# damians13/big-linear-algebra

Hardware: AMD Instinct MI355X
Metric: fp32 GFLOP/s matrix_mul 4096^3 (higher is better)
Workload: dtype f32; 1 GPU; square fp32 matrix_multiply N=4096 (BASELINE configs[1]), operands resident in HBM; kernel=gemm_f32_glds256x256x16_nn_dma_splitk1, parallelism=replicas x1

## Files before the change

big-linear-algebra_amd/csrc/bla_gemm.hip:

```cpp

#include "bla_gemm_kernel.h"

namespace bla {

enum { LOAD_FULL = 0, LOAD_VEC = 1, LOAD_SCALAR = 2 };

template <int ROWS, int COLS, int NT>
struct TileRegs {
	static constexpr int CPR = COLS / 4;
	static constexpr int N = ROWS * COLS / 4 / NT;
	static_assert(ROWS * COLS / 4 % NT == 0, "tile must divide over the workgroup");
	float4 v[N];

	template <int MODE>
	__device__ __forceinline__ void load(const float* __restrict__ g, int ld, int row0, int col0, int row_end, int col_end, int tid) {
#pragma unroll
		for (int i = 0; i < N; i++) {
			int f = tid + i * NT;
			int gr = row0 + f / CPR, gc = col0 + (f % CPR) * 4;
			if (MODE == LOAD_FULL) {
				v[i] = *reinterpret_cast<const float4*>(g + (size_t)gr * ld + gc);
			} else if (MODE == LOAD_VEC) {
				bool ok = gr < row_end && gc < col_end;
				const float* q = g + (size_t)min(gr, row_end - 1) * ld + min(gc, col_end - 4);
// ... 683 lines not shown
			void* ws;
			st = ensure_workspace((size_t)wtiles * ksplit * 1024 * sizeof(float), &ws);
			if (st) return st;
			a.slab = (float*)ws;
		}
		dim3 grid((unsigned)wtiles, (unsigned)ksplit);
		if (plan && ksplit == 1 && avec && bvec) { plan->a = a; plan->akc = akc; plan->bkc = bkc; plan->valid = true; return BLA_OK; }
		hipError_t e = launch_wsk(a, akc, bkc, avec, bvec, grid, s);
		if (e != hipSuccess) return hip_fail(e, "gemm_f32_wsk_kernel launch");
		snprintf(g_last_kernel, sizeof(g_last_kernel), "gemm_f32_wsk%dx%d_%c%c_%s%s_ksplit%d", tile, tile, transa ? 't' : 'n', transb ? 't' : 'n',
		         avec ? "v" : "s", bvec ? "v" : "s", ksplit);
		return BLA_OK;
	}
	BLA_REQUIRE(!a.softmax_grad || cfg == 6, BLA_ERR_INVALID, "fused softmax is only available on the wave-split-K config (6)");
	float* deferred_row_sum = nullptr;
	BLA_REQUIRE(cfg == 6 || !a.row_sum_a || (a.rs_alpha == 1.f && a.rs_beta == 0.f), BLA_ERR_INVALID, "a scaled / accumulated row sum is only available on the wave-split-K config (6)");
	if (cfg != 6 && a.row_sum_a) { deferred_row_sum = a.row_sum_a; a.row_sum_a = nullptr; }
	if (kConfigs[cfg].glds && !(vec_ok && k > 0 && k % kConfigs[cfg].bk == 0)) {
		set_error("gemm config %d (%s) needs 16-byte aligned operands, contiguous extents %% 4 == 0 and k %% %d == 0", cfg,
		          kConfigs[cfg].name, kConfigs[cfg].bk);
		return BLA_ERR_INVALID;
	}
	const Config& c = kConfigs[cfg];
	a.tiles_m = (m + c.bm - 1) / c.bm;
	a.tiles_n = (n + c.bn - 1) / c.bn;
	long tiles = (long)a.tiles_m * a.tiles_n;
	int splits = g_force_split;
	if (splits <= 0) {
		splits = 1;
		if (tiles < cus && k >= 256) {
			long want = (2L * cus + tiles - 1) / tiles;
			long maxs = k / 128;
			splits = (int)(want < maxs ? want : maxs);
			if (splits < 1) splits = 1;
			if (splits > 32) splits = 32;
		}
	}
	if ((cfg >= 11 && cfg <= 15) || cfg == kCfgHs192) {
		BLA_REQUIRE(m % c.bm == 0 && n % c.bn == 0 && k >= 2 * c.bk && ldc % 4 == 0 && (uintptr_t)C % 16 == 0, BLA_ERR_INVALID,
		            "gemm config %d (%s) needs m, n multiples of the tile, k >= %d and a 16-byte aligned C", cfg, c.name, 2 * c.bk);
		a.rc_global = 0;
		BLA_REQUIRE(!a.bias_row && !a.bias_col && !a.pre_act && a.act == BLA_ACT_NONE && !a.relu_mask && a.beta == 0.f && !deferred_row_sum, BLA_ERR_INVALID,
		            "gemm config %d (%s) takes a plain epilogue (alpha only)", cfg, c.name);
		splits = 1;
	}
	if (cfg == 10) {
		BLA_REQUIRE(k % (2 * c.bk) == 0, BLA_ERR_INVALID, "gemm config 10 (%s) needs k %% %d == 0", c.name, 2 * c.bk);
		splits = 1;
	}
	int kps = (k + splits - 1) / splits;
	kps = (kps + c.bk - 1) / c.bk * c.bk;
	if (kps == 0) kps = c.bk;
	splits = k > 0 ? (k + kps - 1) / kps : 1;
	a.k_per_split = kps;
	a.splits = splits;
	a.slab = nullptr;
	if (splits > 1) {
		void* ws;
		st = ensure_workspace((size_t)splits * m * n * sizeof(float), &ws);
		if (st) return st;
		a.slab = (float*)ws;
	}
	int mode = LOAD_SCALAR;
	if (vec_ok) {
		mode = LOAD_VEC;
		if (m % c.bm == 0 && n % c.bn == 0 && k % c.bk == 0) mode = LOAD_FULL;
	}
	dim3 grid((unsigned)tiles, 1, (unsigned)splits);
	hipError_t e;
	switch (cfg) {
		case 0: e = launch_variant<128, 128, 16, 2, 2>(a, akc, bkc, mode, grid, s); break;
		case 1: e = launch_variant<64, 64, 16, 2, 2>(a, akc, bkc, mode, grid, s); break;
		case 2: e = launch_variant<128, 128, 32, 2, 2>(a, akc, bkc, mode, grid, s); break;
		case 3: e = launch_glds<128, 128, 16, 2, 2>(a, akc, bkc, grid, s); break;
		case 4: e = launch_glds<64, 64, 16, 2, 2>(a, akc, bkc, grid, s); break;
		case 5: e = launch_glds<128, 128, 32, 2, 2>(a, akc, bkc, grid, s); break;
		case 7: e = launch_glds<128, 64, 16, 2, 2>(a, akc, bkc, grid, s); break;
		case 8: e = launch_glds<128, 256, 16, 2, 2, 2, 3>(a, akc, bkc, grid, s); break;
		case 9: e = launch_glds<256, 128, 16, 2, 2, 2, 3>(a, akc, bkc, grid, s); break;
		case 10: {
			unsigned tiles = grid.x, cap = 2u * (unsigned)cus;
			e = launch_glds<128, 128, 16, 2, 2, 1, 2, true>(a, akc, bkc, dim3(tiles < cap ? tiles : cap, 1, 1), s);
		} break;
		case 11: e = launch_glds<256, 256, 16, 2, 2>(a, akc, bkc, grid, s); break;
		case 12: e = launch_glds<256, 256, 32, 2, 2>(a, akc, bkc, grid, s); break;
		case 13: e = launch_glds<128, 512, 16, 1, 4>(a, akc, bkc, grid, s); break;
		case 14: e = launch_glds<128, 128, 16, 2, 2, 1, 2, false, true>(a, akc, bkc, grid, s); break;
		case 15: e = launch_glds<128, 256, 16, 2, 2, 1, 2, false, true>(a, akc, bkc, grid, s); break;
		case 18: e = launch_glds<64, 64, 32, 2, 2, 1, 2, false, false, 2>(a, akc, bkc, grid, s); break;
		default: e = launch_glds<192, 192, 16, 2, 2, 1, 2, false, true>(a, akc, bkc, grid, s); break;
	}
	if (e != hipSuccess) return hip_fail(e, "gemm_f32_kernel launch");
	static const char* kModeName[] = {"full", "vec", "scalar"};
	snprintf(g_last_kernel, sizeof(g_last_kernel), "gemm_f32_%s_%c%c_%s_splitk%d", c.name, transa ? 't' : 'n', transb ? 't' : 'n',
	         c.glds ? "dma" : kModeName[mode], splits);
	if (splits > 1) {
		e = launch_splitk_reduce(a, s);
		if (e != hipSuccess) return hip_fail(e, "gemm_splitk_reduce_kernel launch");
	}
	if (deferred_row_sum) return window_sum(stream, A, m, k, lda, deferred_row_sum);
	return BLA_OK;
}

extern "C" {

bla_status bla_gemm_f32(void* stream, int transa, int transb, int m, int n, int k,
                        const float* A, int lda, const float* B, int ldb, float* C, int ldc,
                        const bla_gemm_epilogue* ep) {
	return gemm_impl(stream, transa, transb, m, n, k, A, lda, B, ldb, C, ldc, ep, nullptr);
}

bla_status bla_gemm_pair_f32(void* stream, const bla_gemm_desc* p, const bla_gemm_desc* q) { return gemm_pair_with_hook(stream, p, q, nullptr, nullptr); }

}

bla_status bla::gemm_pair_with_hook(void* stream, const bla_gemm_desc* p, const bla_gemm_desc* q, const DoneHook* d_hook, bool* posted) {
	if (posted) *posted = false;
	BLA_REQUIRE(p && q, BLA_ERR_INVALID, "null descriptor");
	WskPlan pp = {}, pq = {};
	const bool try_pair = g_force_config < 0 && g_force_split <= 0;
	bla_status st = gemm_impl(stream, p->transa, p->transb, p->m, p->n, p->k, p->A, p->lda, p->B, p->ldb, p->C, p->ldc, p->ep, try_pair ? &pp : nullptr);
	if (st) return st;
	st = gemm_impl(stream, q->transa, q->transb, q->m, q->n, q->k, q->A, q->lda, q->B, q->ldb, q->C, q->ldc, q->ep, pp.valid ? &pq : nullptr);
	if (st) return st;
	hipStream_t s = pick_stream(stream);
	const int tp = pp.valid ? pp.a.tiles_m * pp.a.tiles_n : 0, tq = pq.valid ? pq.a.tiles_m * pq.a.tiles_n : 0;
	hipError_t e = hipSuccess;
	if (pp.valid && pq.valid && !pp.a.softmax_grad && !pq.a.softmax_grad) {
		const dim3 grid((unsigned)(tp + tq));
		const int combo = (pp.akc ? 8 : 0) | (pp.bkc ? 4 : 0) | (pq.akc ? 2 : 0) | (pq.bkc ? 1 : 0);
#define BLA_PAIR_CASE(I) case I: hipLaunchKernelGGL((gemm_f32_wsk_pair_kernel<((I) & 8) != 0, ((I) & 4) != 0, ((I) & 2) != 0, ((I) & 1) != 0>), grid, dim3(256), 0, s, pp.a, pq.a, tp, d_hook); break
		switch (combo) {
			BLA_PAIR_CASE(0); BLA_PAIR_CASE(1); BLA_PAIR_CASE(2); BLA_PAIR_CASE(3); BLA_PAIR_CASE(4); BLA_PAIR_CASE(5); BLA_PAIR_CASE(6); BLA_PAIR_CASE(7);
			BLA_PAIR_CASE(8); BLA_PAIR_CASE(9); BLA_PAIR_CASE(10); BLA_PAIR_CASE(11); BLA_PAIR_CASE(12); BLA_PAIR_CASE(13); BLA_PAIR_CASE(14); BLA_PAIR_CASE(15);
		}
#undef BLA_PAIR_CASE
		e = hipGetLastError();
		if (posted && e == hipSuccess) *posted = d_hook != nullptr;
		snprintf(g_last_kernel, sizeof(g_last_kernel), "gemm_f32_wsk_pair_%c%c+%c%c_%dx%d+%dx%d", pp.akc ? 'n' : 't', pp.bkc ? 't' : 'n', pq.akc ? 'n' : 't',
		         pq.bkc ? 't' : 'n', tp, pp.a.wsk_tile, tq, pq.a.wsk_tile);
	} else {
		if (pp.valid) e = launch_wsk(pp.a, pp.akc, pp.bkc, true, true, dim3((unsigned)tp, 1), s);
		if (e == hipSuccess && pq.valid) e = launch_wsk(pq.a, pq.akc, pq.bkc, true, true, dim3((unsigned)tq, 1), s);
	}
	if (e != hipSuccess) return hip_fail(e, "gemm_f32_wsk pair launch");
	return BLA_OK;
}

extern "C" {

bla_status bla_gemm_batched_f32(void* stream, int transa, int transb, int m, int n, int k, const float* A, int lda, long stride_a, const float* B, int ldb,
                                long stride_b, float* C, int ldc, long stride_c, int batch, const bla_gemm_epilogue* ep, long stride_pre) {
	BLA_REQUIRE(batch >= 1, BLA_ERR_INVALID, "batch %d", batch);
	BLA_REQUIRE(!ep || (!ep->relu_mask && !ep->row_sum_a && !ep->softmax_grad), BLA_ERR_INVALID, "batched products take alpha / beta, the biases, act and pre_act only");
	if (batch == 1) return gemm_impl(stream, transa, transb, m, n, k, A, lda, B, ldb, C, ldc, ep, nullptr);
	if (g_force_config < 0 && g_force_split <= 0 && gemm_thin_applies(m, n, k, batch) && (!ep || (!ep->bias_col && ep->act == BLA_ACT_NONE))) {
		BLA_REQUIRE(A && B && C, BLA_ERR_INVALID, "null operand");
		const ThinPart part = {A, B, stride_a, stride_b, lda, ldb};
		bla_status st = gemm_thin_parts(stream, transa, transb, m, n, k, &part, 1, C, ldc, stride_c, batch, ep ? ep->alpha : 1.f, ep ? ep->beta : 0.f,
		                                ep ? ep->bias_row : nullptr, ep ? ep->pre_act : nullptr, ep ? ep->ld_pre : 0, stride_pre);
		if (st == BLA_OK) snprintf(g_last_kernel, sizeof(g_last_kernel), "gemm_f32_thin_%c%c_x%d", transa ? 't' : 'n', transb ? 't' : 'n', batch);
		return st;
	}
	WskPlan pl = {};
	const bool aligned = stride_a % 4 == 0 && stride_b % 4 == 0 && stride_c % 4 == 0 && stride_pre % 4 == 0;
	t_plan_batch = batch;
	bla_status st = gemm_impl(stream, transa, transb, m, n, k, A, lda, B, ldb, C, ldc, ep, g_force_config < 0 && g_force_split <= 0 && aligned ? &pl : nullptr);
// ... 58 lines not shown
```

big-linear-algebra_amd/csrc/bla_gemm_kernel.h:

```cpp
#pragma once
#include "bla_internal.h"
#include <cstdlib>

namespace bla {

typedef float f32x16 __attribute__((ext_vector_type(16)));

struct GemmArgs {
	const float* A; const float* B; float* C;
	int M, N, K, lda, ldb, ldc;
	int tiles_m, tiles_n, k_per_split, splits;
	float* slab;
	float alpha, beta;
	const float* bias_row; const float* bias_col;
	float* pre_act; int ld_pre; int act;
	const float* relu_mask; int ld_mask;
#ifdef BLA_WSK_DIAG
	unsigned long long* stamps;
#endif
	unsigned* counters;
	float* row_sum_a;
	float rs_alpha, rs_beta;
	const float* softmax_y; float softmax_scale; float* softmax_grad;
	double* sm_loss; unsigned* sm_correct;
// ... 264 lines not shown
		if (GATHER == 3) {
#pragma unroll
			for (int i = 0; i < B_NI; i++) {
				const int idx = wave * B_NI + i, kr = idx * 2 + (lane >> 5);
				const float* src = p.g_img + (g3_base + p.g_ktab[g_k + kr].x);
				__builtin_amdgcn_global_load_lds((gbl_ptr_t)src, (lds_ptr_t)(base + A_SZ + idx * 256), 16, 0, 0);
			}
			g_k += BK;
		} else if (GATHER) {
			const int simg = GATHER == 2 ? g_img * p.g_img_stride : 0;
#pragma unroll
			for (int i = 0; i < B_NI; i++) {
				const int idx = wave * B_NI + i, krow = idx >> 1, hf = idx & 1;
				const int2 ts = p.g_ktab[GATHER == 1 ? g_k + krow : g_r + krow];
				const int yy = (short)(g_lyx[hf] & 0xffff) + (short)(ts.y & 0xffff), xx = (g_lyx[hf] >> 16) + (ts.y >> 16);
				const bool ok = g_lval[hf] && (unsigned)yy < (unsigned)p.g_H && (unsigned)xx < (unsigned)p.g_W;
				const float* src = ok ? p.g_img + (g_loff[hf] + ts.x + simg) : p.g_zero;
				__builtin_amdgcn_global_load_lds((gbl_ptr_t)src, (lds_ptr_t)(base + A_SZ + krow * BN + hf * 64), 4, 0, 0);
			}
			g_k += BK;
			if (GATHER == 2) {
				g_r += BK;
				if (g_r >= p.g_HWo) {
					g_r = 0; g_img++;
#pragma unroll
					for (int i = 0; i < A_NI; i++) ga[i] += (size_t)(p.M - 1) * p.g_HWo;
				}
			}
		} else {
#pragma unroll
			for (int i = 0; i < B_NI; i++) {
				__builtin_amdgcn_global_load_lds((gbl_ptr_t)gb[i], (lds_ptr_t)(base + A_SZ + (wave * B_NI + i) * 256), 16, 0, 0);
				gb[i] += b_step;
			}
		}
	};

	f32x16 acc[TM][TN];
#pragma unroll
	for (int i = 0; i < TM; i++)
#pragma unroll
		for (int j = 0; j < TN; j++)
#pragma unroll
			for (int r = 0; r < 16; r++) acc[i][j][r] = 0.f;

	auto frags = [&](const float* As, const float* Bs, int kk, float (&a)[TM][4], float (&b)[TN][4]) {
#pragma unroll
		for (int i = 0; i < TM; i++) {
			if (AKC) {
				float4 x = *reinterpret_cast<const float4*>(As + AI::off(wm0 + i * 32 + l31, kk * 2 + h));
				a[i][0] = x.x; a[i][1] = x.y; a[i][2] = x.z; a[i][3] = x.w;
			} else {
#pragma unroll
				for (int j = 0; j < 4; j++) a[i][j] = As[(kk * 8 + 4 * h + j) * BM + wm0 + i * 32 + l31];
			}
		}
#pragma unroll
		for (int i = 0; i < TN; i++) {
			if (BKC) {
				float4 x = *reinterpret_cast<const float4*>(Bs + BI::off(wn0 + i * 32 + l31, kk * 2 + h));
				b[i][0] = x.x; b[i][1] = x.y; b[i][2] = x.z; b[i][3] = x.w;
			} else {
#pragma unroll
				for (int j = 0; j < 4; j++) b[i][j] = Bs[(kk * 8 + 4 * h + j) * BN + wn0 + i * 32 + l31];
			}
		}
	};

	auto mfma_group = [&](float (&a)[KKW][TM][4], float (&b)[KKW][TN][4], int kk, int j) {
#pragma unroll
		for (int im = 0; im < TM; im++)
#pragma unroll
			for (int in = 0; in < TN; in++)
				acc[im][in] = __builtin_amdgcn_mfma_f32_32x32x2f32(a[kk][im][j], b[kk][in][j], acc[im][in], 0, 0, 0);
	};
	auto rest = [&](float (&pa)[KKW][TM][4], float (&pb)[KKW][TN][4]) {
#pragma unroll
		for (int kk = 0; kk < KKW; kk++)
#pragma unroll
			for (int j = 0; j < 4; j++)
				if (kk != 0 || j != 0) mfma_group(pa, pb, kk, j);
	};
	constexpr bool HALFSLAB = ((TM == 4 && TN == 4) || (HS && TM >= 2 && TM <= 4 && TN >= 2 && TN <= 4)) && (KK == 2 || KK == 4) &&
	                          (GATHER == 0 || ((GATHER == 3 || GATHER == 4 || G7) && HS)) && !PERSIST && NBUF == 2;
	constexpr int NDMA = G7 ? A_NI + 1 : A_NI + B_NI;
	size_t g_adv_a = 0, g_adv_b = 0;
	int w7_tap = 0, w7_g = 0;
	const int w7_groups = G7 ? (p.g_img_stride / p.g_HWo) / 16 : 0, w7_gstep = 16 * p.g_HWo;
	const float* const w7_img = p.g_img;
	const float* const w7_zero = p.g_zero;
#if defined(__HIP_DEVICE_COMPILE__)
	int hs_tap[B_NI][2];
	auto hs_prefetch = [&]() {
		if (GATHER == 3) {
#pragma unroll
			for (int i = 0; i < B_NI; i++) {
				const int row = __builtin_amdgcn_readfirstlane(g_k + (wave * B_NI + i) * G3_RPI);
				hs_tap[i][0] = p.g_ktab[row].x; hs_tap[i][1] = G3_RPI == 2 ? p.g_ktab[row + 1].x : 0;
			}
		}
	};
	if (HALFSLAB && GATHER == 3) hs_prefetch();

	auto dma_one = [&](int buf, int d) {
		float* base = lds + buf * (A_SZ + B_SZ);
		if (d < A_NI) {
			const int i = d;
			if (GATHER == 4) {
				__builtin_amdgcn_raw_ptr_buffer_load_lds(rsrc_img, (lds_ptr_t)(base + (wave * A_NI + i) * 256), 16, g4_voff[i], g4_soff, 0, 0);
			} else if (A_BUF) __builtin_amdgcn_raw_ptr_buffer_load_lds(rsrc_a, (lds_ptr_t)(base + (wave * A_NI + i) * 256), 16, voff_a[i], soff_a, 0, 0);
			else __builtin_amdgcn_global_load_lds((gbl_ptr_t)(ga[i] + g_adv_a), (lds_ptr_t)(base + (wave * A_NI + i) * 256), 16, 0, 0);
		} else if (G7) {
			if (w7_tap < W7_PW && wave + 4 * w7_tap < W7_NI && w7_g + 1 < w7_groups) {
				const int i = w7_tap;
				const int off = window_chunk_offset<W7_PL, GWS>((wave + 4 * i) * 64 + lane, w7_i0, p.g_H, p.g_HWo, w7_base);
				const float* src = off >= 0 ? w7_img + (off + (w7_g + 1) * w7_gstep) : w7_zero;
				float* dst = lds + 2 * A_SZ + 4 + ((w7_g + 1) & 1) * W7_GRP + (wave + 4 * i) * 256;
				__builtin_amdgcn_global_load_lds((gbl_ptr_t)src, (lds_ptr_t)dst, 16, 0, 0);
			}
		} else {
			const int i = d - A_NI;
			if (GATHER == 3) {
				const int idx = wave * B_NI + i;
				const float* src = p.g_img + (g3_base + ((G3_RPI == 2 && (lane >> 5)) ? hs_tap[i][1] : hs_tap[i][0]));
				__builtin_amdgcn_global_load_lds((gbl_ptr_t)src, (lds_ptr_t)(base + A_SZ + idx * 256), 16, 0, 0);
			} else if (B_BUF) __builtin_amdgcn_raw_ptr_buffer_load_lds(rsrc_b, (lds_ptr_t)(base + A_SZ + (wave * B_NI + i) * 256), 16, voff_b[i], soff_b, 0, 0);
			else __builtin_amdgcn_global_load_lds((gbl_ptr_t)(gb[i] + g_adv_b), (lds_ptr_t)(base + A_SZ + (wave * B_NI + i) * 256), 16, 0, 0);
		}
	};
	auto dma_advance = [&](bool really) {
		const int sa = really ? (int)(a_step * 4) : 0, sb = really ? (int)(b_step * 4) : 0;
		if (GATHER == 3) { soff_a += sa; g_k += really ? BK : 0; hs_prefetch(); return; }
		if (G7) { soff_a += sa; return; }
		if (GATHER == 4) {
			const int r1 = g_r + (really ? BK : 0);
			const bool wrap = r1 >= p.g_HWo;
			soff_b += (really ? BK * 4 : 0) + (wrap ? (p.N - 1) * p.g_HWo * 4 : 0);
			g_r = wrap ? 0 : r1; g_img += wrap ? 1 : 0;
			const int c1 = g4_col + 16;
			const bool row_end = c1 >= p.g_wo;
			g4_pix0 = wrap ? 0 : g4_pix0 + (really ? (row_end ? g4_step_end : g4_step) : 0);
			g4_col = (wrap || row_end) ? 0 : (really ? c1 : g4_col);
			g4_soff = __builtin_amdgcn_readfirstlane((g_img * p.g_img_stride + g4_pix0) * 4);
			return;
		}
		if (A_BUF) soff_a += sa; else g_adv_a += really ? a_step : 0;
		if (B_BUF) soff_b += sb; else g_adv_b += really ? b_step : 0;
	};
#else
	auto dma_one = [&](int, int) {};
	auto dma_advance = [&](bool) {};
#endif
	auto step = [&](int kt, bool do_dma, float (&pa)[KKW][TM][4], float (&pb)[KKW][TN][4], float (&qa)[KKW][TM][4], float (&qb)[KKW][TN][4]) {
		mfma_group(pa, pb, 0, 0);
		__builtin_amdgcn_sched_barrier(0);
		asm volatile("s_waitcnt vmcnt(0)" ::: "memory");
		__builtin_amdgcn_s_barrier();
		const float* As = lds + ((kt + 1) & 1) * (A_SZ + B_SZ);
#pragma unroll
		for (int kk = 0; kk < KKW; kk++) frags(As, As + A_SZ, wk * KKW + kk, qa[kk], qb[kk]);
		if (do_dma) dma(kt & 1);
		__builtin_amdgcn_sched_barrier(0);
		rest(pa, pb);
		__builtin_amdgcn_sched_barrier(0);
	};

	auto store_tile = [&]() {
		if (GATHER == 4) {
			float* dst = p.splits > 1 ? p.slab + (size_t)zsplit * p.M * p.N : p.C;
			const int ld = p.splits > 1 ? p.M : p.ldc;
#pragma unroll
			for (int in = 0; in < TN; in++) {
				int col = n0 + wn0 + in * 32 + l31;
				if (col >= p.N) continue;
#pragma unroll
				for (int im = 0; im < TM; im++)
#pragma unroll
					for (int qq = 0; qq < 4; qq++) {
						int row = m0 + wm0 + im * 32 + 8 * qq + 4 * h;
						if (row + 3 < p.M)
							*reinterpret_cast<float4*>(dst + (size_t)col * ld + row) =
								make_float4(acc[im][in][4 * qq], acc[im][in][4 * qq + 1], acc[im][in][4 * qq + 2], acc[im][in][4 * qq + 3]);
					}
			}
			return;
		}
		if constexpr (G7) {
			const int b = n0 / p.g_HWo;
			const size_t img_off = (size_t)b * p.M * p.g_HWo + (n0 - b * p.g_HWo) + wn0 + l31;
			const float* bias = p.g_bias ? p.g_bias + (size_t)b * p.g_bias_stride : nullptr;
#pragma unroll
			for (int im = 0; im < TM; im++)
#pragma unroll
				for (int r = 0; r < 16; r++) {
					const int row = m0 + wm0 + im * 32 + (r & 3) + 8 * (r >> 2) + 4 * h;
					const size_t o = img_off + (size_t)row * p.g_HWo;
					const float bv = bias ? bias[row] : 0.f;
#pragma unroll
					for (int in = 0; in < TN; in++) {
						const float v = acc[im][in][r] + bv;
						p.C[o + in * 32] = v;
						if (p.g_out2) p.g_out2[o + in * 32] = v + p.g_add[o + in * 32];
					}
				}
			return;
		}
		if constexpr (GATHER == 3 && HALFSLAB) {
			const int col = n0 + wn0 + TN * l31;
			const int b = col / p.g_HWo, rr = col - b * p.g_HWo;
			const size_t img_off = (size_t)b * p.M * p.g_HWo + rr;
			float* cbase = (p.splits > 1 ? p.slab + (size_t)zsplit * p.M * p.N : p.C) + img_off;
			const float* bias = p.g_bias ? p.g_bias + (size_t)b * p.g_bias_stride : nullptr;
#pragma unroll
			for (int im = 0; im < TM; im++)
#pragma unroll
				for (int r = 0; r < 16; r++) {
					const int row = m0 + wm0 + im * 32 + (r & 3) + 8 * (r >> 2) + 4 * h;
					const size_t o = (size_t)row * p.g_HWo;
					const float bv = bias ? bias[row] : 0.f;
					if (TN == 4) {
						const float4 v = make_float4(acc[im][0][r] + bv, acc[im][1][r] + bv, acc[im][TN > 2 ? 2 : 0][r] + bv, acc[im][TN > 3 ? 3 : 0][r] + bv);
						*reinterpret_cast<float4*>(cbase + o) = v;
						if (p.g_out2) {
							const float4 a4 = *reinterpret_cast<const float4*>(p.g_add + img_off + o);
							*reinterpret_cast<float4*>(p.g_out2 + img_off + o) = make_float4(v.x + a4.x, v.y + a4.y, v.z + a4.z, v.w + a4.w);
						}
					} else {
						const float2 v = make_float2(acc[im][0][r] + bv, acc[im][1][r] + bv);
						*reinterpret_cast<float2*>(cbase + o) = v;
						if (p.g_out2) {
							const float2 a2 = *reinterpret_cast<const float2*>(p.g_add + img_off + o);
							*reinterpret_cast<float2*>(p.g_out2 + img_off + o) = make_float2(v.x + a2.x, v.y + a2.y);
						}
					}
				}
			return;
		}
		if (GATHER == 1 || GATHER == 3) {
#pragma unroll
			for (int in = 0; in < TN; in++) {
				int col = n0 + wn0 + in * 32 + l31;
				if (col >= p.N) continue;
				int b = col / p.g_HWo, r = col - b * p.g_HWo;
				float* cbase = p.C + (size_t)b * p.M * p.g_HWo + r;
#pragma unroll
				for (int im = 0; im < TM; im++)
#pragma unroll
					for (int q = 0; q < 16; q++) {
						int row = m0 + wm0 + im * 32 + (q & 3) + 8 * (q >> 2) + 4 * h;
// ... 162 lines not shown
					__builtin_amdgcn_sched_barrier(0);
#pragma unroll
					for (int m = FRONT ? u : u * NM / NU; m < (FRONT ? (u + 1 < NU ? u + 1 : NM) : (u + 1) * NM / NU); m++) mf1(use, m);
					__builtin_amdgcn_sched_barrier(0);
				}
			}
			land(Q);
			asm volatile("s_waitcnt vmcnt(0)" ::: "memory");
			__builtin_amdgcn_s_barrier();
#if defined(__HIP_DEVICE_COMPILE__)
			if constexpr (GATHER == 3) {
#pragma unroll
				for (int i = 0; i < B_NI; i++) { asm volatile("" : "+v"(hs_tap[i][0])); if (G3_RPI == 2) asm volatile("" : "+v"(hs_tap[i][1])); }
			}
#endif
			constexpr int PER = 2 * (NU + NDMA) <= NM ? 2 : 1;
			static_assert(PER * (NU + NDMA) <= NM, "too many memory instructions for the MFMAs of one k-part");
#pragma unroll
			for (int u = 0; u < NU; u++) {
				read_unit(nxt, 0, u, P);
				__builtin_amdgcn_sched_barrier(0);
#pragma unroll
				for (int m = 0; m < PER; m++) mf1(Q, PER * u + m);
				__builtin_amdgcn_sched_barrier(0);
			}
#pragma unroll
			for (int d = 0; d < NDMA; d++) {
				dma_one(t & 1, d);
				__builtin_amdgcn_sched_barrier(0);
#pragma unroll
				for (int m = 0; m < PER; m++) mf1(Q, PER * (NU + d) + m);
				__builtin_amdgcn_sched_barrier(0);
			}
			{ const bool adv = fetched + 1 < nkt; dma_advance(adv); fetched += adv ? 1 : 0; }
#pragma unroll
			for (int m = PER * (NU + NDMA); m < NM; m++) mf1(Q, m);
			__builtin_amdgcn_sched_barrier(0);
			if constexpr (G7) { const bool wrap = w7_tap == 8; w7_g += wrap ? 1 : 0; w7_tap = wrap ? 0 : w7_tap + 1; }
		};
		auto mf_fs = [&](Frag (&f)[KK], int idx) {
			mf1(f[idx / NM], idx % NM);
		};
		auto slab_fs = [&](int t, Frag (&use)[KK], Frag (&fill)[KK]) {
			const unsigned nxt = ((t + 1) & 1) * BUF_BYTES;
			if constexpr (G7) {
				const int tap1 = w7_tap == 8 ? 0 : w7_tap + 1, g1 = w7_tap == 8 ? w7_g + 1 : w7_g;
				w7_cur = (t & 1) * BUF_BYTES; w7_ad[0] = w7_addr(w7_g, w7_tap); w7_ad[1] = w7_addr(g1, tap1);
			}
			asm volatile("s_waitcnt lgkmcnt(0)" ::: "memory");
#pragma unroll
			for (int kk = 0; kk < KK; kk++) land(use[kk]);
			asm volatile("s_waitcnt vmcnt(0)" ::: "memory");
			__builtin_amdgcn_s_barrier();
#if defined(__HIP_DEVICE_COMPILE__)
			if constexpr (GATHER == 3) {
#pragma unroll
				for (int i = 0; i < B_NI; i++) { asm volatile("" : "+v"(hs_tap[i][0])); if (G3_RPI == 2) asm volatile("" : "+v"(hs_tap[i][1])); }
			}
#endif
			static_assert(!FS || KK * NU + NDMA <= KK * NM, "one memory instruction per MFMA");
			int idx = 0;
#pragma unroll
			for (int kk = 0; kk < KK; kk++)
#pragma unroll
				for (int u = 0; u < NU; u++) {
					read_unit(nxt, kk, u, fill[kk]);
					__builtin_amdgcn_sched_barrier(0);
					mf_fs(use, idx++);
					__builtin_amdgcn_sched_barrier(0);
				}
#pragma unroll
			for (int d = 0; d < NDMA; d++) {
				dma_one(t & 1, d);
				__builtin_amdgcn_sched_barrier(0);
				mf_fs(use, idx++);
				__builtin_amdgcn_sched_barrier(0);
			}
			{ const bool adv = fetched + 1 < nkt; dma_advance(adv); fetched += adv ? 1 : 0; }
#pragma unroll
			for (int m = KK * NU + NDMA; m < KK * NM; m++) mf_fs(use, m);
			__builtin_amdgcn_sched_barrier(0);
			if constexpr (G7) { const bool wrap = w7_tap == 8; w7_g += wrap ? 1 : 0; w7_tap = wrap ? 0 : w7_tap + 1; }
		};
		if (nkt > 0) {
			if constexpr (G7) {
#if defined(__HIP_DEVICE_COMPILE__)
#pragma unroll
				for (int i = 0; i < W7_PW; i++)
					if (wave + 4 * i < W7_NI) {
						const int off = window_chunk_offset<W7_PL, GWS>((wave + 4 * i) * 64 + lane, w7_i0, p.g_H, p.g_HWo, w7_base);
						const float* src = off >= 0 ? w7_img + off : w7_zero;
						__builtin_amdgcn_global_load_lds((gbl_ptr_t)src, (lds_ptr_t)(lds + 2 * A_SZ + 4 + (wave + 4 * i) * 256), 16, 0, 0);
					}
#endif
				w7_cur = 0; w7_ad[0] = w7_addr(0, 0);
			}
			fetch_slab(0);
			fetch_slab(1);
			asm volatile("s_waitcnt vmcnt(0)" ::: "memory");
			__builtin_amdgcn_s_barrier();
			if constexpr (FS) {
#pragma unroll
				for (int kk = 0; kk < KK; kk++)
#pragma unroll
					for (int u = 0; u < NU; u++) read_unit(0, kk, u, F0[kk]);
				int t = 0;
				for (; t + 1 < nkt; t += 2) { slab_fs(t, F0, F1); slab_fs(t + 1, F1, F0); }
				if (t < nkt) slab_fs(t, F0, F1);
			} else {
#pragma unroll
				for (int u = 0; u < NU; u++) read_unit(0, 0, u, P);
				for (int t = 0; t < nkt; t++) slab(t);
			}
			asm volatile("s_waitcnt vmcnt(0)" ::: "memory");
		}
		store_tile();
		return;
	}

	if constexpr (PERSIST) {
		static_assert(NBUF == 2, "persistent pipeline uses the two-buffer scheme");
		const int total = p.tiles_m * p.tiles_n;
		const float* gan[A_NI];
		const float* gbn[B_NI];
		int dma_left = nkt;
		auto dma_next = [&](int buf) {
			const bool sw = dma_left == 0;
#pragma unroll
			for (int i = 0; i < A_NI; i++) ga[i] = sw ? gan[i] : ga[i];
#pragma unroll
			for (int i = 0; i < B_NI; i++) gb[i] = sw ? gbn[i] : gb[i];
			dma_left = (sw ? nkt : dma_left) - 1;
			dma(buf);
		};
		auto plan_next = [&](int vb_next) {
			int tm0, tn0;
			tile_origin(vb_next < total ? vb_next : blk_x, tm0, tn0);
			const float* sa[A_NI]; const float* sb[B_NI];
#pragma unroll
			for (int i = 0; i < A_NI; i++) sa[i] = ga[i];
#pragma unroll
			for (int i = 0; i < B_NI; i++) sb[i] = gb[i];
			open_tile(tm0, tn0);
#pragma unroll
			for (int i = 0; i < A_NI; i++) { gan[i] = ga[i]; ga[i] = sa[i]; }
#pragma unroll
			for (int i = 0; i < B_NI; i++) { gbn[i] = gb[i]; gb[i] = sb[i]; }
		};
		float fa0[KK][TM][4], fb0[KK][TN][4], fa1[KK][TM][4], fb1[KK][TN][4];
		auto pstep = [&](int cur, float (&pa)[KK][TM][4], float (&pb)[KK][TN][4], float (&qa)[KK][TM][4], float (&qb)[KK][TN][4]) {
			mfma_group(pa, pb, 0, 0);
			__builtin_amdgcn_sched_barrier(0);
			asm volatile("s_waitcnt vmcnt(0)" ::: "memory");
			__builtin_amdgcn_s_barrier();
			const float* As = lds + (cur ^ 1) * (A_SZ + B_SZ);
#pragma unroll
			for (int kk = 0; kk < KK; kk++) frags(As, As + A_SZ, kk, qa[kk], qb[kk]);
			dma_next(cur);
			__builtin_amdgcn_sched_barrier(0);
			rest(pa, pb);
			__builtin_amdgcn_sched_barrier(0);
		};
		if (nkt > 0 && blk_x < total) {
			dma_next(0);
			asm volatile("s_waitcnt vmcnt(0)" ::: "memory");
			__builtin_amdgcn_s_barrier();
#pragma unroll
			for (int kk = 0; kk < KK; kk++) frags(lds, lds + A_SZ, kk, fa0[kk], fb0[kk]);
			dma_next(1);
			for (int vb = blk_x; vb < total; vb += grid_x) {
				tile_origin(vb, m0, n0);
				plan_next(vb + grid_x);
				__builtin_amdgcn_sched_barrier(0);
				for (int kt = 0; kt < nkt; kt += 2) {
					pstep(0, fa0, fb0, fa1, fb1);
					pstep(1, fa1, fb1, fa0, fb0);
				}
				store_tile();
#pragma unroll
				for (int i = 0; i < TM; i++)
#pragma unroll
					for (int j = 0; j < TN; j++)
#pragma unroll
						for (int r = 0; r < 16; r++) acc[i][j][r] = 0.f;
				__builtin_amdgcn_sched_barrier(0);
			}
		}
		return;
	}

	if constexpr (NBUF == 3) {
		static_assert(KK == 2, "split-fragment pipeline is written for BK = 16");
		{ float agpr_hint = 0.f; asm volatile("; keep accumulators in AGPRs %0" ::"a"(agpr_hint)); }
		float xa[TM][4], xb[TN][4], ya[TM][4], yb[TN][4], za[TM][4], zb[TN][4];
		auto mf = [&](float (&a)[TM][4], float (&b)[TN][4], int j) {
#pragma unroll
			for (int im = 0; im < TM; im++)
#pragma unroll
				for (int in = 0; in < TN; in++) acc[im][in] = __builtin_amdgcn_mfma_f32_32x32x2f32(a[im][j], b[in][j], acc[im][in], 0, 0, 0);
// ... 106 lines not shown
```

Measured before the change: 150,400 GFLOP/s.

## Add multi-buffer tail epilogue overlapping C stores with final slabs for 256x256 tile

Switches the 256x256x16 glds config to four LDS buffers and enables the half-slab path with NBUF>2 for 4x4 wave tiles. The last slabs are prefetched into extra buffers at kernel start, and a dedicated tail loop interleaves the final MFMAs with nontemporal row stores of finished accumulator groups. The aim is to hide the epilogue store cost behind the remaining compute. In exchange it needs more LDS, which may lower occupancy, and it adds a complex new store path that bypasses store_tile (alpha only, no beta, split-k or bias handling).

Result: no change. 150,900 GFLOP/s (median of 6 runs) (+0.4%).

```diff
diff --git a/big-linear-algebra_amd/csrc/bla_gemm.hip b/big-linear-algebra_amd/csrc/bla_gemm.hip
--- a/big-linear-algebra_amd/csrc/bla_gemm.hip
+++ b/big-linear-algebra_amd/csrc/bla_gemm.hip
@@ -789,7 +789,7 @@
 			unsigned tiles = grid.x, cap = 2u * (unsigned)cus;
 			e = launch_glds<128, 128, 16, 2, 2, 1, 2, true>(a, akc, bkc, dim3(tiles < cap ? tiles : cap, 1, 1), s);
 		} break;
-		case 11: e = launch_glds<256, 256, 16, 2, 2>(a, akc, bkc, grid, s); break;
+		case 11: e = launch_glds<256, 256, 16, 2, 2, 1, 4>(a, akc, bkc, grid, s); break;
 		case 12: e = launch_glds<256, 256, 32, 2, 2>(a, akc, bkc, grid, s); break;
 		case 13: e = launch_glds<128, 512, 16, 1, 4>(a, akc, bkc, grid, s); break;
 		case 14: e = launch_glds<128, 128, 16, 2, 2, 1, 2, false, true>(a, akc, bkc, grid, s); break;
diff --git a/big-linear-algebra_amd/csrc/bla_gemm_kernel.h b/big-linear-algebra_amd/csrc/bla_gemm_kernel.h
--- a/big-linear-algebra_amd/csrc/bla_gemm_kernel.h
+++ b/big-linear-algebra_amd/csrc/bla_gemm_kernel.h
@@ -370,7 +370,9 @@
 				if (kk != 0 || j != 0) mfma_group(pa, pb, kk, j);
 	};
 	constexpr bool HALFSLAB = ((TM == 4 && TN == 4) || (HS && TM >= 2 && TM <= 4 && TN >= 2 && TN <= 4)) && (KK == 2 || KK == 4) &&
-	                          (GATHER == 0 || ((GATHER == 3 || GATHER == 4 || G7) && HS)) && !PERSIST && NBUF == 2;
+	                          (GATHER == 0 || ((GATHER == 3 || GATHER == 4 || G7) && HS)) && !PERSIST &&
+	                          (NBUF == 2 || (NBUF > 2 && GATHER == 0 && TM == 4 && TN == 4 && KK == 2));
+	constexpr int TAIL = HALFSLAB && NBUF > 2 ? NBUF : 0;
 	constexpr int NDMA = G7 ? A_NI + 1 : A_NI + B_NI;
 	size_t g_adv_a = 0, g_adv_b = 0;
 	int w7_tap = 0, w7_g = 0;
@@ -435,9 +437,19 @@
 		if (A_BUF) soff_a += sa; else g_adv_a += really ? a_step : 0;
 		if (B_BUF) soff_b += sb; else g_adv_b += really ? b_step : 0;
 	};
+	auto fetch_at = [&](int buf, int s) {
+		const int sa0 = soff_a, sb0 = soff_b;
+		const size_t ga0 = g_adv_a, gb0 = g_adv_b;
+		if (A_BUF) soff_a = s * (int)(a_step * 4); else g_adv_a = (size_t)s * a_step;
+		if (B_BUF) soff_b = s * (int)(b_step * 4); else g_adv_b = (size_t)s * b_step;
+#pragma unroll
+		for (int d = 0; d < NDMA; d++) dma_one(buf, d);
+		soff_a = sa0; soff_b = sb0; g_adv_a = ga0; g_adv_b = gb0;
+	};
 #else
 	auto dma_one = [&](int, int) {};
 	auto dma_advance = [&](bool) {};
+	auto fetch_at = [&](int, int) {};
 #endif
 	auto step = [&](int kt, bool do_dma, float (&pa)[KKW][TM][4], float (&pb)[KKW][TN][4], float (&qa)[KKW][TM][4], float (&qb)[KKW][TN][4]) {
 		mfma_group(pa, pb, 0, 0);
@@ -453,6 +465,21 @@
 		__builtin_amdgcn_sched_barrier(0);
 	};
 
+	auto store_row = [&](int im, int r) {
+		const int i = (r & 3) + 8 * (r >> 2) + 4 * h;
+		const int row = m0 + wm0 + ((AKC || TM == 3) ? im * 32 + i : TM * i + im);
+		float* cp = p.C + (size_t)row * p.ldc + n0 + wn0;
+		if (BKC || TN == 3) {
+#pragma unroll
+			for (int in = 0; in < TN; in++) __builtin_nontemporal_store(p.alpha * acc[im][in][r], cp + in * 32 + l31);
+		} else if (TN == 4) {
+			typedef float nt4 __attribute__((ext_vector_type(4)));
+			const nt4 v = {p.alpha * acc[im][0][r], p.alpha * acc[im][1][r], p.alpha * acc[im][TN > 2 ? 2 : 0][r], p.alpha * acc[im][TN > 3 ? 3 : 0][r]};
+			__builtin_nontemporal_store(v, reinterpret_cast<nt4*>(cp + 4 * l31));
+		} else {
+			*reinterpret_cast<float2*>(cp + 2 * l31) = make_float2(p.alpha * acc[im][0][r], p.alpha * acc[im][1][r]);
+		}
+	};
 	auto store_tile = [&]() {
 		if (GATHER == 4) {
 			float* dst = p.splits > 1 ? p.slab + (size_t)zsplit * p.M * p.N : p.C;
@@ -781,6 +808,50 @@
 			__builtin_amdgcn_sched_barrier(0);
 			if constexpr (G7) { const bool wrap = w7_tap == 8; w7_g += wrap ? 1 : 0; w7_tap = wrap ? 0 : w7_tap + 1; }
 		};
+		constexpr int NUA = AKC ? 1 : UA, NUT = NUA + UB;
+		constexpr unsigned AGRP = AKC ? 32 * BK * 4 : 0;
+		auto tail_read = [&](unsigned abuf, unsigned bbuf, int g, int kk, int u, Frag& f) {
+			if (u < NUA) {
+				if constexpr (AKC) asm volatile("ds_read_b128 %0, %1 offset:%2" : "=v"(f.ka[0]) : "v"(abuf + a_ad[kk]), "n"(g * 32 * BK * 4));
+				else read_unit(abuf, kk, u, f);
+			} else read_unit(bbuf, kk, UA + u - NUA, f);
+		};
+		auto tail_phase = [&](Frag& use, int g, Frag& fill, unsigned abuf, unsigned bbuf, int gf, int kf, int sg, int r0) {
+#pragma unroll
+			for (int m = 0; m < 4 * TN; m++) {
+				if (m < NUT) tail_read(abuf, bbuf, gf, kf, m, fill);
+				if (sg >= 0 && (m & 1)) store_row(sg, r0 + m / 2);
+				__builtin_amdgcn_sched_barrier(0);
+				const int j = m / TN, in = m % TN;
+				acc[g][in] = __builtin_amdgcn_mfma_f32_32x32x2f32(AKC ? use.ka[0][j] : use.ra[j][g], opb(use, in, j), acc[g][in], 0, 0, 0);
+				__builtin_amdgcn_sched_barrier(0);
+			}
+		};
+		auto tail = [&](int ns) {
+			const int t0 = nkt - ns;
+			auto sbuf = [&](int i) -> unsigned { return (unsigned)(i < 2 ? ((t0 + i) & 1) : i) * BUF_BYTES; };
+#pragma unroll
+			for (int g = 0; g < TM; g++) {
+				land(P);
+				tail_phase(P, g, Q, sbuf(0), sbuf(0), g, 1, g - 1, 0);
+				land(Q);
+				if (g == 0) {
+					asm volatile("s_waitcnt vmcnt(0)" ::: "memory");
+					__builtin_amdgcn_s_barrier();
+				}
+				tail_phase(Q, g, P, sbuf(1), sbuf(1), g, 0, g - 1, 8);
+				for (int s = 1; s < ns; s++) {
+					land(P);
+					tail_phase(P, g, Q, sbuf(s), sbuf(s), g, 1, -1, 0);
+					land(Q);
+					const bool last = s + 1 == ns;
+					const unsigned nb = last ? sbuf(0) : sbuf(s + 1);
+					tail_phase(Q, g, P, nb + (last ? AGRP : 0u), nb, g, 0, -1, 0);
+				}
+			}
+#pragma unroll
+			for (int r = 0; r < 16; r++) store_row(TM - 1, r);
+		};
 		if (nkt > 0) {
 			if constexpr (G7) {
 #if defined(__HIP_DEVICE_COMPILE__)
@@ -796,7 +867,11 @@
 			}
 			fetch_slab(0);
 			fetch_slab(1);
-			asm volatile("s_waitcnt vmcnt(0)" ::: "memory");
+			if constexpr (TAIL) {
+#pragma unroll
+				for (int i = 2; i < TAIL; i++) fetch_at(i, min(nkt - min(TAIL, nkt) + i, nkt - 1));
+				asm volatile("s_waitcnt vmcnt(%0)" ::"n"((TAIL - 1) * NDMA) : "memory");
+			} else asm volatile("s_waitcnt vmcnt(0)" ::: "memory");
 			__builtin_amdgcn_s_barrier();
 			if constexpr (FS) {
 #pragma unroll
@@ -809,11 +884,13 @@
 			} else {
 #pragma unroll
 				for (int u = 0; u < NU; u++) read_unit(0, 0, u, P);
-				for (int t = 0; t < nkt; t++) slab(t);
-			}
-			asm volatile("s_waitcnt vmcnt(0)" ::: "memory");
-		}
-		store_tile();
+				const int ns = TAIL ? min(TAIL, nkt) : 0;
+				for (int t = 0; t < nkt - ns; t++) slab(t);
+				if constexpr (TAIL) tail(ns);
+			}
+			if constexpr (!TAIL) asm volatile("s_waitcnt vmcnt(0)" ::: "memory");
+		}
+		if constexpr (!TAIL) store_tile();
 		return;
 	}
 
```
